# bjzhb666/GS-LoRA

Measured on AMD Instinct MI355X. Metric: forgetting-step images/sec, ViT-P8S8 d6 112px r=8, higher is better.
Workload: dtype fp16

## Files before the change

### gs-lora_amd/csrc/attention.hip

```cpp
#include <stdlib.h>

#include <algorithm>
#include <type_traits>

#include "gsl_common.h"

using namespace gsl;
#include "gsl_h16.h"
GSL_OPNS_BEGIN

typedef op16x8_t bf16x8_t;
typedef __attribute__((ext_vector_type(4))) float f32x4_t;

constexpr int HD = 64;
constexpr int KLD = 80;
__device__ __forceinline__ int lds_off(int row, int col) { return row * KLD + col; }

union Frag {
  uint4 u;
  uint2 h[2];
  bf16x8_t v;
};

__device__ __forceinline__ f32x4_t mfma16(const bf16x8_t a, const bf16x8_t b, const f32x4_t c) {
// ... 1973 lines not shown
  GSL_CHECK_ARG(qkv && o && d_o_cls && lse && dqkv && B > 0 && T > 1 && H > 0, "null/size");
  GSL_CHECK_ARG(qkv_layout >= 0 && qkv_layout <= 2 && (qkv_layout != 2 || (q_cls && dq_cls)), "qkv_layout: 0 token-major, 1 head-major, 2 kv + q_cls / dq_cls");
  const dim3 grid(B * H), blk(256);
  if (dtype == GSL_OP16)
    hipLaunchKernelGGL(attn_bwd_cls_kernel<bf16_t>, grid, blk, 0, as_stream(s), (const bf16_t*)qkv, (const bf16_t*)q_cls, (const bf16_t*)o,
                       (const bf16_t*)d_o_cls, lse, (bf16_t*)dqkv, (bf16_t*)dq_cls, T, H, scale, qkv_layout, cls_compact);
#if GSL_HAS_F32
  else if (dtype == GSL_F32)
    hipLaunchKernelGGL(attn_bwd_cls_kernel<float>, grid, blk, 0, as_stream(s), (const float*)qkv, (const float*)q_cls, (const float*)o,
                       (const float*)d_o_cls, lse, (float*)dqkv, (float*)dq_cls, T, H, scale, qkv_layout, cls_compact);
#endif
  else return fail(GSL_ERR_ARG, "gsl_attention_bwd_cls: bad dtype%s %ld", "", dtype);
  return check_launch("gsl_attention_bwd_cls");
}

#ifdef GSL_DEV
static inline int attn_env(const char* name, int dflt) { const char* e = getenv(name); return e ? atoi(e) : dflt; }
static inline unsigned long long* attn_stamps() { const char* sp = getenv("GSL_ATTN_STAMPS"); return sp ? reinterpret_cast<unsigned long long*>(strtoull(sp, nullptr, 0)) : nullptr; }
#else
static inline constexpr int attn_env(const char*, int dflt) { return dflt; }
static inline constexpr unsigned long long* attn_stamps() { return nullptr; }
#endif
static inline int attn_persistent() { return attn_env("GSL_ATTN_PERSISTENT", 1); }
static inline int attn_num_cus() {
  static int n = 0;
  if (!n) {
    int dev = 0; hipDeviceProp_t pr;
    if (hipGetDevice(&dev) == hipSuccess && hipGetDeviceProperties(&pr, dev) == hipSuccess && pr.multiProcessorCount > 0) n = pr.multiProcessorCount;
    else n = 256;
  }
// ... 127 lines not shown
```

### gs-lora_amd/csrc/gsl_h16.h

```cpp
#pragma once
#include "gsl_common.h"

extern "C" {
int h16_gsl_gemm_nt(const void* A1, int lda1, const void* W1, int ldw1, int K1, const void* A2, int lda2, const void* W2, int ldw2, int K2,
                    int M, int N, int dtype, int epilogue, float alpha, const float* bias, const void* res, const void* aux, void* out,
                    void* out2, int ldo, const float* pos, const float* cls, int T, float p_drop, uint64_t seed, uint32_t site, gsl_stream_t s);
int h16_gsl_gemm_nt_lora(const void* A, int lda, const void* W, int ldw, int K, const void* P, int ldp, const void* Q, int ldq,
                         float lora_scale, void* tout, int ldt, int M, int N, int dtype, int epilogue, const float* bias, const void* res,
                         const void* aux, void* out, void* out2, int ldo, float p_drop, uint64_t seed, uint32_t site, gsl_stream_t s);
int h16_gsl_gemm_nt_lora_mulgrad(const void* A, int lda, const void* W, int ldw, int K, const void* P, int ldp, const void* Q, int ldq,
                                 float lora_scale, void* tout, int ldt, int M, int N, const void* aux, void* out, int ldo, const void* U1,
                                 int ldu1, float* G1, long g1sn, long g1sj, const void* Y2, float* G2, long g2sn, long g2sj, int r,
                                 int accumulate, float* ws, int aux_u8, float p_drop, int dtype, const float* gscale, gsl_stream_t s);
int h16_gsl_attention_fwd(const void* qkv, void* o, float* lse, int B, int T, int H, float scale, int dtype, int qkv_layout, gsl_stream_t s);
int h16_gsl_attention_bwd(const void* qkv, const void* o, const void* d_o, const float* lse, void* dqkv, float* delta_ws, int B, int T,
                          int H, float scale, int dtype, int qkv_layout, gsl_stream_t s);
int h16_gsl_attention_fwd_cls(const void* qkv, const void* q_cls, void* o_cls, float* lse_cls, int B, int T, int H, float scale, int dtype,
                              int qkv_layout, gsl_stream_t s);
int h16_gsl_attention_bwd_cls(const void* qkv, const void* q_cls, const void* o, const void* d_o_cls, const float* lse, void* dqkv,
                              void* dq_cls, int B, int T, int H, float scale, int dtype, int qkv_layout, int cls_compact, gsl_stream_t s);
}

#ifdef GSL_OP_F16
#define GSL_FORWARD_H16(dtype, call)
#define GSL_HAS_F32 0
#else
#define GSL_FORWARD_H16(dtype, call) do { if ((dtype) == GSL_F16) return call; } while (0)
#define GSL_HAS_F32 1
#endif
```

### gs-lora_amd/gslora_hip/_lib.py

```python
import ctypes as C
import os

import contextlib

_HERE = os.path.dirname(os.path.abspath(__file__))
LIB_PATH = os.environ.get("GSLORA_HIP_LIB") or os.path.join(_HERE, "libgslora_hip.so")
DEV_LIB_PATH = os.path.join(_HERE, "libgslora_hip_dev.so")

F32, BF16, F16 = 0, 1, 2
EPI_STORE, EPI_BIAS_RES_F32, EPI_BIAS_GELU, EPI_MUL, EPI_PATCH, EPI_STORE_F32, EPI_STORE_QKV_HM, EPI_BIAS_RES_BF16, EPI_PATCH_BF16 = 0, 1, 2, 3, 4, 5, 6, 7, 8
EPI_MUL_G8, EPI_BIAS_GELU_G8, EPI_BIAS_RES_F16, EPI_PATCH_F16, EPI_STORE_LN, EPI_STORE_QKV_HM_LN = 9, 10, 11, 12, 13, 14
VERIF_FLIP_SUM, VERIF_PLAIN = 0, 1
U8_NCHW, U8_NHWC = 0, 1
NORM_SPLIT = 8
SEED_ON_DEVICE = 0x80000000

_vp, _i, _l, _f, _d, _u64, _u32 = C.c_void_p, C.c_int, C.c_long, C.c_float, C.c_double, C.c_uint64, C.c_uint32

SIGNATURES = {
    "gsl_version": [],
    "gsl_last_error": [],
    "gsl_patchify": [_vp, _vp, _i, _i, _i, _i, _i, _i, _vp],
    "gsl_unfold_patches": [_vp, _vp, _i, _i, _i, _i, _i, _i, _i, _i, _i, _vp],
    "gsl_patchify_u8": [_vp, _i, _vp, _vp, _i, _i, _i, _i, _i, _i, _vp],
    "gsl_unfold_patches_u8": [_vp, _i, _vp, _vp, _i, _i, _i, _i, _i, _i, _i, _i, _i, _vp],
    "gsl_gemm_nt": [_vp, _i, _vp, _i, _i, _vp, _i, _vp, _i, _i, _i, _i, _i, _i, _f, _vp, _vp, _vp, _vp, _vp, _i,
                    _vp, _vp, _i, _f, _u64, _u32, _vp],
    "gsl_gemm_nt_lora": [_vp, _i, _vp, _i, _i, _vp, _i, _vp, _i, _f, _vp, _i, _i, _i, _i, _i, _vp, _vp, _vp, _vp, _vp, _i,
                         _f, _u64, _u32, _vp],
    "gsl_gemm_mulgrad_ws_elems": [_i, _i, _i],
    "gsl_gemm_nt_lora_mulgrad": [_vp, _i, _vp, _i, _i, _vp, _i, _vp, _i, _f, _vp, _i, _i, _i, _vp, _vp, _i,
                                 _vp, _i, _vp, _l, _l, _vp, _vp, _l, _l, _i, _i, _vp, _i, _f, _i, _vp, _vp],
    "gsl_layernorm_fwd": [_vp, _l, _vp, _vp, _f, _vp, _vp, _vp, _i, _i, _i, _i, _vp],
    "gsl_layernorm_fwd_lora": [_vp, _l, _vp, _vp, _f, _vp, _vp, _vp, _i, _i, _vp, _i, _f, _vp, _vp],
    "gsl_layernorm_bwd": [_vp, _vp, _l, _vp, _vp, _vp, _vp, _vp, _l, _vp, _i, _i, _i, _i, _i, _f, _u64, _u32, _l, _i, _vp, _vp],
    "gsl_attention_fwd": [_vp, _vp, _vp, _i, _i, _i, _f, _i, _i, _vp],
    "gsl_attention_bwd": [_vp, _vp, _vp, _vp, _vp, _vp, _i, _i, _i, _f, _i, _i, _vp],
    "gsl_attention_fwd_cls": [_vp, _vp, _vp, _vp, _i, _i, _i, _f, _i, _i, _vp],
    "gsl_attention_bwd_cls": [_vp, _vp, _vp, _vp, _vp, _vp, _vp, _i, _i, _i, _f, _i, _i, _i, _vp],
    "gsl_lora_grad_ws_elems": [_i, _i, _i],
    "gsl_lora_grad": [_vp, _l, _vp, _i, _vp, _l, _l, _i, _i, _i, _i, _i, _vp, _vp, _vp],
    "gsl_lora_grad_batch_ws_elems": [_vp, _i],
    "gsl_lora_grad_batch": [_vp, _i, _vp, _i, _vp, _vp],
    "gsl_cosface_prep": [_vp, _vp, _i, _i, _vp],
    "gsl_head_fwd": [_vp, _i, _i, _vp, _vp, _f, _vp, _vp, _vp, _vp, _vp, _vp, _i, _i, _i, _f, _f, _vp, _i, _i, _vp],
    "gsl_head_bwd": [_vp, _vp, _vp, _i, _i, _vp, _vp, _vp, _vp, _vp, _vp, _vp, _i, _i, _i, _f, _i, _i, _f, _u64, _u32, _i, _i, _i, _vp, _vp, _i, _vp],
    "gsl_head_fwd_margin": [_vp, _i, _i, _vp, _vp, _f, _vp, _vp, _vp, _vp, _vp, _vp, _i, _i, _i, _f, _f, _vp, _i, _i, _i, _d, _i, _vp, _vp],
    "gsl_head_bwd_margin": [_vp, _vp, _vp, _i, _i, _vp, _vp, _vp, _vp, _vp, _vp, _vp, _i, _i, _i, _f, _i, _i, _f, _u64, _u32, _i, _i, _i, _vp,
                            _vp, _i, _i, _d, _i, _vp, _vp, _vp],
    "gsl_ce_fwd": [_vp, _vp, _vp, _vp, _i, _i, _vp],
    "gsl_ce_bwd": [_vp, _vp, _vp, _f, _vp, _i, _i, _i, _vp],
    "gsl_proto_kl_fwd": [_vp, _vp, _vp, _vp, _vp, _i, _i, _i, _vp],
    "gsl_loss_combine": [_vp, _vp, _vp, _vp, _vp, _vp, _vp, _f, _f, _f, _f, _f, _f, _f, _f, _vp, _vp, _vp, _vp],
    "gsl_loss_combine_pack": [_vp, _vp, _i, _f, _f, _f, _f, _f, _f, _vp, _vp, _vp, _vp],
# ... 77 lines not shown
```

### gs-lora_amd/gslora_hip/ops.py

```python
import ctypes

import torch

from . import _lib as L

ATTN_MAX_T = 1025


def check_num_tokens(model, T):
    if T > ATTN_MAX_T:
        raise NotImplementedError(f"{model}: this geometry gives {T} tokens per image; the gs-lora_amd attention kernels take at most "
                                  f"{ATTN_MAX_T} (GSL_ATTN_MAX_T: a 32 x 32 patch grid plus the cls token)")


DT = {torch.float32: L.F32, torch.bfloat16: L.BF16, torch.float16: L.F16}


def _p(t):
    return None if t is None else t.data_ptr()


def _stream():
    return torch.cuda.current_stream().cuda_stream

# ... 271 lines not shown
                                           _stream()), "gsl_attention_fwd_cls")
    return o, lse


def attention_bwd_cls(qkv, o, d_o_cls, lse, B, T, H, scale, layout=0, q_cls=None):
    _need(qkv, o, d_o_cls, lse, q_cls)
    nw = 2 if layout == 2 else 3
    dqkv = torch.empty(B * T, nw * H * 64, device=qkv.device, dtype=qkv.dtype)
    dq = torch.empty(B, H * 64, device=qkv.device, dtype=qkv.dtype) if layout == 2 else None
    compact = o.shape[0] == B and lse.dim() == 2
    L.check(L.load().gsl_attention_bwd_cls(_p(qkv), _p(q_cls), _p(o), _p(d_o_cls), _p(lse), _p(dqkv), _p(dq), B, T, H, float(scale),
                                           code(qkv.dtype), int(layout), 1 if compact else 0, _stream()), "gsl_attention_bwd_cls")
    return (dqkv, dq) if layout == 2 else dqkv




def lora_grad(Y, U, G, gsn, gsj, r, accumulate=True, gscale=None):
    if not (Y.is_cuda and U.is_cuda and Y.stride(1) == 1 and U.stride(1) == 1):
        raise RuntimeError("lora_grad: operands must be CUDA tensors with unit column stride")
    M, N = Y.shape
    lib = L.load()
    need = lib.gsl_lora_grad_ws_elems(M, N, r)
    ws = _workspace((Y.device.index,), need, Y.device, floor=1 << 22)
    L.check(lib.gsl_lora_grad(_p(Y), Y.stride(0), _p(U), U.stride(0), G.data_ptr(), gsn, gsj, M, N, r, code(Y.dtype),
                              1 if accumulate else 0, _p(ws), _p(gscale), _stream()), "gsl_lora_grad")


class _LgradDesc(ctypes.Structure):
    _fields_ = [("Y", ctypes.c_void_p), ("ldy", ctypes.c_long), ("U", ctypes.c_void_p), ("ldu", ctypes.c_int), ("M", ctypes.c_int),
# ... 435 lines not shown
```

### gs-lora_amd/gslora_hip/vit_runner.py

```python
import os

import torch

from . import _lib as L
from . import ops

PADK = 64
OP16 = (torch.bfloat16, torch.float16)
SITE_EMB = 1_000_000
GRAD_STREAM_BF16 = os.environ.get("GSLORA_GRAD_STREAM", "bf16").lower() != "f32"
FWD_STREAM = os.environ.get("GSLORA_FWD_STREAM", "f16").lower()
if FWD_STREAM not in ("f16", "bf16", "f32"):
    raise ValueError(f"GSLORA_FWD_STREAM must be f16, bf16 or f32, not {FWD_STREAM!r}")
GP8 = os.environ.get("GSLORA_GP8", "1") != "0"

FUSE_LORA_GRAD = True
TAIL_CLS = True
QSPLIT = True
INK_MIN_ROWS = 8192
LN1_FOLD = os.environ.get("GSLORA_LN1_FOLD", "1") != "0"
GRAD_TARGET_EXP = int(os.environ.get("GSLORA_GRAD_TARGET_EXP", "0"))
if GRAD_TARGET_EXP and not 4 <= GRAD_TARGET_EXP <= 15:
    raise ValueError(f"GSLORA_GRAD_TARGET_EXP={GRAD_TARGET_EXP}: 0 (default) or 4 .. 15")
INK_SMALL = True
LGRAD_BATCH_MAX_ROWS = 1 << 30
LN_LORA = False
QKV_HEAD_MAJOR = True


class BlockSpec:
    __slots__ = ("ln1", "qkv_w", "qkv_b", "out", "ln2", "l1", "l2", "qkv_lora")

    def __init__(self, ln1, qkv_w, qkv_b, out, ln2, l1, l2, qkv_lora=None):
# ... 186 lines not shown

    def w(self, name, param, dtype):
        if dtype == torch.float32:
            return param.detach()
        return self._cached(self._wcache, (name, "n", dtype), param, lambda p: ops.cast(p.contiguous(), dtype))

    def w_ln(self, name, weight, gamma, beta, bias, dtype):
        def build(weight, gamma, beta, bias=None):
            w32 = weight.float()
            wf = ops.cast((w32 * gamma.float()[None, :]).contiguous(), dtype)
            c = wf.float().sum(1).contiguous()
            d = (w32 @ beta.float()) + (bias.float() if bias is not None else 0.0)
            return wf, c, d.contiguous()
        return self._cached(self._wcache, (name, "ln", dtype), (weight, gamma, beta) + (() if bias is None else (bias,)), build)

    def w_conv(self, name, param, dtype):
        def build(p):
            w2 = p.permute(0, 2, 3, 1).reshape(p.shape[0], -1).contiguous()
            return w2 if dtype == torch.float32 else ops.cast(w2, dtype)
        return self._cached(self._wcache, (name, "conv", dtype), param, build)

    def w_kpad(self, name, param, kpad, dtype):
        def build(p):
            w2 = torch.zeros(p.shape[0], kpad, device=p.device, dtype=torch.float32)
            w2[:, :p.shape[1]] = p
            return w2 if dtype == torch.float32 else ops.cast(w2, dtype)
        return self._cached(self._wcache, (name, "kpad", kpad, dtype), param, build)

    def wT(self, name, param, dtype):
        return self._cached(self._wcache, (name, "t", dtype), param, lambda p: ops.transpose_cast(p.contiguous(), dtype))
# ... 92 lines not shown
            self._lcache.clear()
            self._retired.extend(t[0] for t in self._pack_tables.values())
            self._retired.extend(e["out"] for e in self._packs.values())
            self._packs.clear()
            self._pack_tables.clear()
        return self.bucket

    def forward(self, img, label, save):
        c, parts, u8tab, label = self._fwd_prepare(img, label, save)
        sp = c.sp
        x = self._fwd_patch(c, parts, u8tab)
        stash = []
        for i, blk in enumerate(sp.blocks):
            tail = TAIL_CLS and i == len(sp.blocks) - 1 and sp.pool == "cls"
            xn, mean1, rstd1 = self._fwd_ln1(c, blk, x)
            qkv, q_cls, uq, hm = self._fwd_qkv(c, i, blk, x, xn, mean1, rstd1, tail)
            xn_keep = xn if (c.attn_site and save) else None
            del xn
            o, lse, x1 = self._fwd_attention(c, i, blk, x, qkv, q_cls, hm, tail)
            x2, st = self._fwd_ffn(c, i, blk, x1)
            if save:
                st.update(x=x, mean1=mean1, rstd1=rstd1, qkv=qkv, qkv_hm=hm, o=o, lse=lse, x1=x1, xn=xn_keep, uq=uq, tail=tail, q_cls=q_cls)
                stash.append(st)
            x = x2
        logits, emb, head = self._fwd_head(c, x, label)
        return logits, emb, (dict(ctx=c, layers=stash, x_last=x, emb=emb, label=label, **head) if save else None)

    def _fwd_prepare(self, img, label, save):
        m = self.model
        raw = list(img) if isinstance(img, (tuple, list)) else [img]
        norm = getattr(m, "input_norm", None)
        u8 = norm is not None and all(t.dtype == torch.uint8 for t in raw)
        if norm is not None and not u8 and any(t.dtype == torch.uint8 for t in raw):
            raise ValueError(f"{type(m).__name__}: the batches of one forward must be all uint8 or all float once set_input_norm() is in effect")
        parts = raw if u8 else [t.float().contiguous() for t in raw]
        img = parts[0]
        if not all(t.is_cuda for t in parts):
# ... 69 lines not shown
        kv, q = slice(inner, None), slice(None, inner)
        epi = L.EPI_STORE_LN if fold else L.EPI_STORE
        ops.gemm_nt(a, w[kv], qkv, epilogue=epi, aux=rows(cw, kv), bias=rows(b, kv), **ln)
        q_cls = torch.empty(B, inner, device=c.dev, dtype=dt)
        ops.gemm_nt(a.view(B, T * D)[:, :D], w[q], q_cls, epilogue=epi, T=T if fold else 0,
                    aux=rows(cw, q), bias=rows(b, q), **ln)
        return qkv, q_cls, None, 2

    def _fwd_attention(self, c, i, blk, x, qkv, q_cls, hm, tail):
        sp, B, T, D = c.sp, c.B, c.T, c.D
        if tail:
            o, lse = ops.attention_fwd_cls(qkv, B, T, c.H, sp.attn_scale, layout=hm, q_cls=q_cls)
            xres = x.view(B, T, D)[:, 0].contiguous()
        else:
            o, lse = ops.attention_fwd(qkv, B, T, c.H, sp.attn_scale, layout=hm)
            xres = x
        x1 = torch.empty(xres.shape[0], D, device=c.dev, dtype=c.xdt)
        ops.gemm_nt(o, self.w(f"wo{i}", blk.out.weight, c.dt), x1, epilogue=c.epi_res,
                    bias=blk.out.bias.detach(), res=xres, p_drop=c.p_drop, seed=c.seed, site=(4 * i) | c.sflag)
        return o, lse, x1

    def _fwd_ffn(self, c, i, blk, x1):
        dt, D, r, s_lora, dev, save = c.dt, c.D, c.r, c.s_lora, c.dev, c.save
        p_drop, seed, sflag = c.p_drop, c.seed, c.sflag
        n2, l1, l2 = blk.ln2, blk.l1, blk.l2
        Mr, mlp = x1.shape[0], l1.weight.shape[0]
        lora_on = r > 0 and not c.attn_site and not l1.merged
        ln_u1 = LN_LORA and lora_on and r <= 16 and D in (512, 768) and x1.dtype == torch.bfloat16 and dt == torch.bfloat16
        if ln_u1:
            xn2, mean2, rstd2, u1_ln = ops.layernorm_fwd_lora(x1, D, Mr, D, n2.weight.detach(), n2.bias.detach(), c.eps,
                                                               self.lora_pack(f"A1_{i}", l1.lora_A, "A_rows", dt), s_lora)
        else:
            xn2, mean2, rstd2 = ops.layernorm_fwd(x1, D, Mr, D, n2.weight.detach(), n2.bias.detach(), c.eps, dt)
        if lora_on and (abs(l1.scaling * r - 1.0) > 1e-9 or abs(l2.scaling * r - 1.0) > 1e-9):
            raise NotImplementedError("gs-lora_amd: the fused LoRA path uses scaling = 1 / r (lora_alpha = 1, the only value GS-LoRA "
# ... 204 lines not shown

    def _bwd_ln2(self, c, i, blk, st, dxn2, dx, gather):
        gamma, kw = blk.ln2.weight.detach(), dict(p_drop=c.p_drop, seed=c.seed, site=(4 * i) | c.sflag, gmax=c.gmax)
        if gather:
            return ops.layernorm_bwd(dxn2, st["x1"], c.T * c.D, gamma, _cls_rows(c, st["mean2"].view(-1, 1), 1).view(-1),
                                     _cls_rows(c, st["rstd2"].view(-1, 1), 1).view(-1), dx, drop_row_stride=c.T * c.D, **kw)
        return ops.layernorm_bwd(dxn2, st["x1"], c.D, gamma, st["mean2"], st["rstd2"], dx, **kw)

    def _bwd_attention(self, c, st, d_o, sparse):
        if sparse:
            return ops.attention_bwd_cls(st["qkv"], st["o"], d_o, st["lse"], c.B, c.T, c.H, c.sp.attn_scale, layout=st["qkv_hm"], q_cls=st["q_cls"])
        return ops.attention_bwd(st["qkv"], st["o"], d_o, st["lse"], c.B, c.T, c.H, c.sp.attn_scale, layout=st["qkv_hm"])

    def _bwd_qkv_frozen(self, c, i, blk, st, d_o, sparse):
        dt, D, inner = c.dt, c.D, c.H * 64
        dxn1 = torch.empty(c.M, D, device=c.dev, dtype=dt)
        dqkv = self._bwd_attention(c, st, d_o, sparse)
        wt = self.wT(f"qkv{i}", blk.qkv_w, dt)
        if st["q_cls"] is None:
            ops.gemm_nt(dqkv, wt, dxn1)
        else:
            dkv, dq_cls = dqkv
            ops.gemm_nt(dkv, wt[:, inner:], dxn1)
            rows = dxn1.view(c.B, c.T * D)[:, :D]
            ops.gemm_nt(dq_cls, wt[:, :inner], rows, epilogue=_res_epilogue(dt), bias=self._zeros(D, c.dev), res=rows)
        return dxn1

    def _bwd_qkv_lora(self, c, i, blk, st, dqkv):
        dt, D, r, ml = c.dt, c.D, c.r, blk.qkv_lora
        qo = self.qkv_lora_ops(i, ml, dt)
        v = torch.empty(c.M, PADK, device=c.dev, dtype=dt)
        ops.gemm_nt(dqkv, qo["BblkT"], v, alpha=c.s_lora)
        ng, inner = len(ml.enable_lora), c.H * 64
# ... 11 lines not shown
```

### include/gslora_hip.h

```cpp
#ifndef GSLORA_HIP_H
#define GSLORA_HIP_H

#include <stdint.h>

#ifdef __cplusplus
extern "C" {
#endif

#define GSL_API __attribute__((visibility("default")))

typedef void* gsl_stream_t;

enum gsl_dtype { GSL_F32 = 0, GSL_BF16 = 1, GSL_F16 = 2 };

enum gsl_status {
  GSL_OK = 0,
  GSL_ERR_ARG = -1,
  GSL_ERR_LAUNCH = -2,
  GSL_ERR_UNSUPPORTED = -3
};

enum gsl_epilogue {
  GSL_EPI_STORE = 0,
  GSL_EPI_BIAS_RES_F32 = 1,
// ... 54 lines not shown
GSL_API int gsl_layernorm_fwd_lora(const void* x, long x_row_stride, const float* gamma, const float* beta, float eps, void* y,
                           float* mean, float* rstd, int M, int D, const void* P, int ldp, float alpha, void* u, gsl_stream_t s);
GSL_API int gsl_layernorm_bwd(const void* dy, const void* x, long x_row_stride, const float* gamma,
                      const float* mean, const float* rstd, const void* dres,
                      void* dx, long io_row_stride, void* dxb, int M, int D, int dtype, int stream_dtype, int x_dtype,
                      float p_drop, uint64_t seed, uint32_t site, long drop_row_stride, int dres_cls_T, float* gmax, gsl_stream_t s);

#define GSL_ATTN_MAX_T 1025
GSL_API int gsl_attention_fwd(const void* qkv, void* o, float* lse, int B, int T, int H, float scale, int dtype, int qkv_layout, gsl_stream_t s);
GSL_API int gsl_attention_bwd(const void* qkv, const void* o, const void* d_o, const float* lse, void* dqkv,
                      float* delta_ws, int B, int T, int H, float scale, int dtype, int qkv_layout, gsl_stream_t s);
GSL_API int gsl_attention_fwd_cls(const void* qkv, const void* q_cls, void* o_cls, float* lse_cls, int B, int T, int H, float scale,
                                  int dtype, int qkv_layout, gsl_stream_t s);
GSL_API int gsl_attention_bwd_cls(const void* qkv, const void* q_cls, const void* o, const void* d_o_cls, const float* lse, void* dqkv,
                                  void* dq_cls, int B, int T, int H, float scale, int dtype, int qkv_layout, int cls_compact, gsl_stream_t s);

GSL_API long gsl_lora_grad_ws_elems(int M, int N, int r);
GSL_API int gsl_lora_grad(const void* Y, long ldy, const void* U, int ldu, float* G, long gsn, long gsj,
                  int M, int N, int r, int dtype, int accumulate, float* ws, const float* gscale, gsl_stream_t s);
typedef struct gsl_lgrad_desc {
  const void* Y; long ldy; const void* U; int ldu; int M; int N; int r; int accumulate; int pad_; float* G; long gsn, gsj;
} gsl_lgrad_desc;
GSL_API long gsl_lora_grad_batch_ws_elems(const gsl_lgrad_desc* descs, int n);
GSL_API int gsl_lora_grad_batch(const gsl_lgrad_desc* descs, int n, float* ws, int dtype, const float* gscale, gsl_stream_t s);


GSL_API int gsl_cosface_prep(const float* W, float* Wn, int C, int D, gsl_stream_t s);
GSL_API int gsl_head_fwd(const void* x, int x_dtype, int T, const float* gamma, const float* beta, float eps,
                 const float* Wn, const int64_t* label, float* emb, float* mean, float* rstd,
                 float* logits, int B, int D, int C, float cos_s, float cos_m,
// ... 96 lines not shown
```

Before: 45710.

## Stream last-block CLS attention by folding K/V projections into query and output

For the tail block, where only the CLS token's output is needed, the K and V projections over all tokens are no longer materialized. The CLS query is instead projected through the K weights into model space, scored directly against the layer-normed input, softmaxed, and the probability-weighted row sum is projected through V. The backward pass mirrors this with a dedicated kernel that forms dxn via split hi/lo fp16 MFMA products. This removes the full QKV GEMM and the attention over all tokens in the last block, at the cost of new block-diagonal weight caches, extra small GEMMs, and fp16 hi/lo splitting to limit precision loss.

```diff
diff --git a/gs-lora_amd/csrc/attention.hip b/gs-lora_amd/csrc/attention.hip
--- a/gs-lora_amd/csrc/attention.hip
+++ b/gs-lora_amd/csrc/attention.hip
@@ -2011,6 +2011,297 @@
   return check_launch("gsl_attention_bwd_cls");
 }
 
+constexpr int CS_NT = 256, CS_NW = CS_NT / 64;
+constexpr int CS_TM = 224;
+constexpr int CS_DMAX = 768;
+
+__device__ __forceinline__ void cs_norm8(const uint4 u, float mu, float rs, const float4 g0, const float4 g1, const float4 b0, const float4 b1,
+                                         float v[8]) {
+  unpack2o(u.x, v[0], v[1]); unpack2o(u.y, v[2], v[3]); unpack2o(u.z, v[4], v[5]); unpack2o(u.w, v[6], v[7]);
+  v[0] = fmaf((v[0] - mu) * rs, g0.x, b0.x); v[1] = fmaf((v[1] - mu) * rs, g0.y, b0.y);
+  v[2] = fmaf((v[2] - mu) * rs, g0.z, b0.z); v[3] = fmaf((v[3] - mu) * rs, g0.w, b0.w);
+  v[4] = fmaf((v[4] - mu) * rs, g1.x, b1.x); v[5] = fmaf((v[5] - mu) * rs, g1.y, b1.y);
+  v[6] = fmaf((v[6] - mu) * rs, g1.z, b1.z); v[7] = fmaf((v[7] - mu) * rs, g1.w, b1.w);
+}
+
+constexpr float CS_LO = 256.0f;
+__device__ __forceinline__ void cs_split2(float a, float b, uint32_t& hi, uint32_t& lo) {
+  hi = pack2o(a, b);
+  float ha, hb;
+  unpack2o(hi, ha, hb);
+  lo = pack2o((a - ha) * CS_LO, (b - hb) * CS_LO);
+}
+__device__ __forceinline__ void cs_split8(const float v[8], uint4& hi, uint4& lo) {
+  cs_split2(v[0], v[1], hi.x, lo.x); cs_split2(v[2], v[3], hi.y, lo.y);
+  cs_split2(v[4], v[5], hi.z, lo.z); cs_split2(v[6], v[7], hi.w, lo.w);
+}
+
+__device__ __forceinline__ void cs_rows_dot(const op16_t* __restrict__ xb, const float* __restrict__ mean, const float* __restrict__ rstd,
+                                            const float* __restrict__ gamma, const float* __restrict__ beta, const op16_t* __restrict__ vec,
+                                            int Tn, int D, int H, float* zs) {
+  const int lane = threadIdx.x & 63, wave = threadIdx.x >> 6, fr = lane & 15, fc = lane >> 4;
+  const int ntile = (Tn + 15) >> 4;
+  for (int tile = wave; tile < ntile; tile += CS_NW) {
+    const int t = min(tile * 16 + fr, Tn - 1);
+    const float mu = mean[t], rs = rstd[t];
+    const op16_t* xr = xb + (size_t)t * D + fc * 8;
+    const op16_t* vr = vec + (size_t)min(fr, H - 1) * D + fc * 8;
+    f32x4_t acc = {0.f, 0.f, 0.f, 0.f}, acl = {0.f, 0.f, 0.f, 0.f};
+#pragma unroll 4
+    for (int k = 0; k < D; k += 32) {
+      const uint4 xv = *reinterpret_cast<const uint4*>(xr + k);
+      const float4* gp = reinterpret_cast<const float4*>(gamma + k + fc * 8);
+      const float4* bp = reinterpret_cast<const float4*>(beta + k + fc * 8);
+      float v[8];
+      cs_norm8(xv, mu, rs, gp[0], gp[1], bp[0], bp[1], v);
+      Frag a, al, b;
+      cs_split8(v, a.u, al.u);
+      b.u = *reinterpret_cast<const uint4*>(vr + k);
+      if (fr >= H) b.u = make_uint4(0, 0, 0, 0);
+      acc = mfma16(a.v, b.v, acc);
+      acl = mfma16(al.v, b.v, acl);
+    }
+    acc += acl * (1.0f / CS_LO);
+#pragma unroll
+    for (int i = 0; i < 4; ++i) zs[fr * CS_TM + tile * 16 + 4 * fc + i] = acc[i];
+  }
+}
+
+template <int HP>
+__device__ __forceinline__ void cs_weighted_rowsum(const op16_t* __restrict__ xb, const float* __restrict__ mean, const float* __restrict__ rstd,
+                                                   const float* __restrict__ gamma, const float* __restrict__ beta, const float* w, float* red,
+                                                   op16_t* __restrict__ out, int Tn, int D, int H) {
+  const int lane = threadIdx.x & 63, wave = threadIdx.x >> 6;
+  const int C = D >> 3;
+  for (int c0 = 0; c0 < C; c0 += 64) {
+    const int c = c0 + lane;
+    const bool live = c < C;
+    const int cc = live ? c : 0;
+    const float4 g0 = *reinterpret_cast<const float4*>(gamma + cc * 8), g1 = *reinterpret_cast<const float4*>(gamma + cc * 8 + 4);
+    const float4 b0 = *reinterpret_cast<const float4*>(beta + cc * 8), b1 = *reinterpret_cast<const float4*>(beta + cc * 8 + 4);
+    float acc[HP][8];
+#pragma unroll
+    for (int h = 0; h < HP; ++h)
+#pragma unroll
+      for (int i = 0; i < 8; ++i) acc[h][i] = 0.f;
+#pragma unroll 2
+    for (int t = wave; t < Tn; t += CS_NW) {
+      const uint4 xv = *reinterpret_cast<const uint4*>(xb + (size_t)t * D + cc * 8);
+      float v[8];
+      cs_norm8(xv, mean[t], rstd[t], g0, g1, b0, b1, v);
+      const float4* wr = reinterpret_cast<const float4*>(w + t * 16);
+#pragma unroll
+      for (int h4 = 0; h4 < HP / 4; ++h4) {
+        const float4 wv = wr[h4];
+        const float ws[4] = {wv.x, wv.y, wv.z, wv.w};
+#pragma unroll
+        for (int j = 0; j < 4; ++j)
+#pragma unroll
+          for (int i = 0; i < 8; ++i) acc[h4 * 4 + j][i] = fmaf(ws[j], v[i], acc[h4 * 4 + j][i]);
+      }
+    }
+#pragma unroll
+    for (int h = 0; h < HP; ++h) {
+      __syncthreads();
+      *reinterpret_cast<float4*>(red + wave * 512 + lane * 8) = make_float4(acc[h][0], acc[h][1], acc[h][2], acc[h][3]);
+      *reinterpret_cast<float4*>(red + wave * 512 + lane * 8 + 4) = make_float4(acc[h][4], acc[h][5], acc[h][6], acc[h][7]);
+      __syncthreads();
+      if (wave == (h & (CS_NW - 1)) && live && h < H) {
+        float s[8];
+#pragma unroll
+        for (int i = 0; i < 8; ++i) s[i] = red[lane * 8 + i];
+#pragma unroll
+        for (int wv = 1; wv < CS_NW; ++wv)
+#pragma unroll
+          for (int i = 0; i < 8; ++i) s[i] += red[wv * 512 + lane * 8 + i];
+        *reinterpret_cast<uint4*>(out + (size_t)h * D + c * 8) =
+            make_uint4(pack2o(s[0], s[1]), pack2o(s[2], s[3]), pack2o(s[4], s[5]), pack2o(s[6], s[7]));
+      }
+    }
+    __syncthreads();
+  }
+}
+
+template <int HP>
+__global__ __launch_bounds__(CS_NT) void attn_cls_stream_fwd_kernel(const op16_t* __restrict__ x, const float* __restrict__ mean,
+                                                                    const float* __restrict__ rstd, const float* __restrict__ gamma,
+                                                                    const float* __restrict__ beta, const op16_t* __restrict__ qt,
+                                                                    const float* __restrict__ sb, op16_t* __restrict__ y, float* __restrict__ p,
+                                                                    int Tn, int D, int H) {
+  GSL_OP16_KERNEL_ENTRY();
+  __shared__ __align__(16) float zs[16 * CS_TM];
+  __shared__ __align__(16) float pt[CS_TM * 16];
+  __shared__ __align__(16) float red[CS_NW * 512];
+  const int b = blockIdx.x, lane = threadIdx.x & 63, wave = threadIdx.x >> 6;
+  const op16_t* xb = x + (size_t)b * Tn * D;
+  const float* mb = mean + (size_t)b * Tn;
+  const float* rb = rstd + (size_t)b * Tn;
+  for (int i = threadIdx.x; i < CS_TM * 16; i += CS_NT) pt[i] = 0.f;
+  cs_rows_dot(xb, mb, rb, gamma, beta, qt + (size_t)b * H * D, Tn, D, H, zs);
+  __syncthreads();
+  for (int h = wave; h < H; h += CS_NW) {
+    const float add = sb ? sb[(size_t)b * H + h] : 0.f;
+    float s[4], m = -3.0e38f;
+#pragma unroll
+    for (int j = 0; j < 4; ++j) {
+      const int t = lane + 64 * j;
+      s[j] = t < Tn ? zs[h * CS_TM + t] + add : -3.0e38f;
+      m = fmaxf(m, s[j]);
+    }
+    m = wave_max(m);
+    float e = 0.f;
+#pragma unroll
+    for (int j = 0; j < 4; ++j) { s[j] = (lane + 64 * j < Tn) ? expf(s[j] - m) : 0.f; e += s[j]; }
+    e = wave_sum(e);
+    const float inv = 1.0f / e;
+#pragma unroll
+    for (int j = 0; j < 4; ++j) {
+      const int t = lane + 64 * j;
+      if (t < Tn) {
+        const float pv = s[j] * inv;
+        p[((size_t)b * H + h) * Tn + t] = pv;
+        pt[t * 16 + h] = pv;
+      }
+    }
+  }
+  __syncthreads();
+  cs_weighted_rowsum<HP>(xb, mb, rb, gamma, beta, pt, red, y + (size_t)b * H * D, Tn, D, H);
+}
+
+constexpr int CS_DC = 256;
+constexpr int CS_BWD_AB = CS_TM * 32 * 2, CS_BWD_R1 = (16 * CS_TM + CS_TM * 16 + CS_NW * 512) * 4;
+static_assert(CS_DC * 32 * 2 <= CS_BWD_R1, "the [qt ; dy]^T pass fits the retired region");
+constexpr int CS_BWD_LDS = 2 * CS_BWD_AB + CS_BWD_R1;
+
+template <int HP>
+__global__ __launch_bounds__(CS_NT) void attn_cls_stream_bwd_kernel(const op16_t* __restrict__ x, const float* __restrict__ mean,
+                                                                    const float* __restrict__ rstd, const float* __restrict__ gamma,
+                                                                    const float* __restrict__ beta, const op16_t* __restrict__ qt,
+                                                                    const float* __restrict__ p, const op16_t* __restrict__ dy,
+                                                                    op16_t* __restrict__ dqt, op16_t* __restrict__ dxn, int Tn, int D, int H) {
+  GSL_OP16_KERNEL_ENTRY();
+  extern __shared__ __align__(16) unsigned char cs_smem[];
+  op16_t* ab = reinterpret_cast<op16_t*>(cs_smem);
+  op16_t* abl = reinterpret_cast<op16_t*>(cs_smem + CS_BWD_AB);
+  float* zs = reinterpret_cast<float*>(cs_smem + 2 * CS_BWD_AB);
+  float* dst = zs + 16 * CS_TM;
+  float* red = dst + CS_TM * 16;
+  op16_t* bt = reinterpret_cast<op16_t*>(cs_smem + 2 * CS_BWD_AB);
+  const int b = blockIdx.x, lane = threadIdx.x & 63, wave = threadIdx.x >> 6, fr = lane & 15, fc = lane >> 4;
+  const op16_t* xb = x + (size_t)b * Tn * D;
+  const float* mb = mean + (size_t)b * Tn;
+  const float* rb = rstd + (size_t)b * Tn;
+  for (int i = threadIdx.x; i < CS_TM * 16; i += CS_NT) {
+    dst[i] = 0.f;
+    reinterpret_cast<uint32_t*>(ab)[i] = 0u;
+    reinterpret_cast<uint32_t*>(abl)[i] = 0u;
+  }
+  cs_rows_dot(xb, mb, rb, gamma, beta, dy + (size_t)b * H * D, Tn, D, H, zs);
+  __syncthreads();
+  for (int h = wave; h < H; h += CS_NW) {
+    float pv[4], dp[4], c = 0.f;
+#pragma unroll
+    for (int j = 0; j < 4; ++j) {
+      const int t = lane + 64 * j;
+      pv[j] = t < Tn ? p[((size_t)b * H + h) * Tn + t] : 0.f;
+      dp[j] = t < Tn ? zs[h * CS_TM + t] : 0.f;
+      c = fmaf(pv[j], dp[j], c);
+    }
+    c = wave_sum(c);
+#pragma unroll
+    for (int j = 0; j < 4; ++j) {
+      const int t = lane + 64 * j;
+      if (t < Tn) {
+        const float ds = pv[j] * (dp[j] - c);
+        dst[t * 16 + h] = ds;
+        uint32_t hi, lo;
+        cs_split2(ds, pv[j], hi, lo);
+        ab[t * 32 + h] = (op16_t)(hi & 0xffffu); ab[t * 32 + 16 + h] = (op16_t)(hi >> 16);
+        abl[t * 32 + h] = (op16_t)(lo & 0xffffu); abl[t * 32 + 16 + h] = (op16_t)(lo >> 16);
+      }
+    }
+  }
+  __syncthreads();
+  cs_weighted_rowsum<HP>(xb, mb, rb, gamma, beta, dst, red, dqt + (size_t)b * H * D, Tn, D, H);
+  const int ntile = (Tn + 15) >> 4;
+  for (int d0 = 0; d0 < D; d0 += CS_DC) {
+    const int dc = min(CS_DC, D - d0), Cc = dc >> 3;
+    __syncthreads();
+    for (int idx = threadIdx.x; idx < 32 * Cc; idx += CS_NT) {
+      const int k = idx / Cc, c = idx - k * Cc, hh = k & 15;
+      uint4 u = make_uint4(0, 0, 0, 0);
+      if (hh < H) u = *reinterpret_cast<const uint4*>((k < 16 ? qt : dy) + ((size_t)b * H + hh) * D + d0 + c * 8);
+      const uint32_t w4[4] = {u.x, u.y, u.z, u.w};
+#pragma unroll
+      for (int i = 0; i < 4; ++i) {
+        bt[(c * 8 + 2 * i) * 32 + k] = (op16_t)(w4[i] & 0xffffu);
+        bt[(c * 8 + 2 * i + 1) * 32 + k] = (op16_t)(w4[i] >> 16);
+      }
+    }
+    __syncthreads();
+    for (int tile = wave; tile < ntile; tile += CS_NW) {
+      const int t = tile * 16 + fr;
+      const bf16x8_t bhi = *reinterpret_cast<const bf16x8_t*>(ab + (tile * 16 + fr) * 32 + fc * 8);
+      const bf16x8_t blo = *reinterpret_cast<const bf16x8_t*>(abl + (tile * 16 + fr) * 32 + fc * 8);
+      op16_t* orow = dxn + ((size_t)b * Tn + min(t, Tn - 1)) * D + d0 + 4 * fc;
+#pragma unroll 4
+      for (int dtile = 0; dtile < (dc >> 4); ++dtile) {
+        const bf16x8_t afrag = *reinterpret_cast<const bf16x8_t*>(bt + (dtile * 16 + fr) * 32 + fc * 8);
+        const f32x4_t z = {0.f, 0.f, 0.f, 0.f};
+        f32x4_t acc = mfma16(afrag, bhi, z);
+        acc += mfma16(afrag, blo, z) * (1.0f / CS_LO);
+        if (t < Tn) store4bf(orow + dtile * 16, acc, 1.0f);
+      }
+    }
+  }
+}
+
+__global__ __launch_bounds__(256) void attn_cls_stream_sb_kernel(const op16_t* __restrict__ q_cls, const float* __restrict__ bk,
+                                                                 float* __restrict__ sb, int n, int H, float scale) {
+  GSL_OP16_KERNEL_ENTRY();
+  const int i = blockIdx.x * 256 + threadIdx.x;
+  if (i >= n) return;
+  const op16_t* q = q_cls + (size_t)i * HD;
+  const float* bb = bk + (size_t)(i % H) * HD;
+  float s = 0.f;
+  for (int j = 0; j < HD; ++j) s = fmaf(o2f(q[j]), bb[j], s);
+  sb[i] = s * scale;
+}
+
+#define GSL_CLS_STREAM_ARGS "16-bit dtype, 2 <= T <= 224, 1 <= H <= 16, D % 64 == 0, D <= 768"
+extern "C" int GSL_ENTRY(gsl_attention_cls_stream_sb)(const void* q_cls, const float* bk, float* sb, int B, int H, float scale, int dtype,
+                                                      gsl_stream_t s) {
+  GSL_FORWARD_H16(dtype, h16_gsl_attention_cls_stream_sb(q_cls, bk, sb, B, H, scale, dtype, s));
+  GSL_CHECK_ARG(q_cls && bk && sb && B > 0 && H > 0 && dtype == GSL_OP16, "null/size/16-bit dtype");
+  hipLaunchKernelGGL(attn_cls_stream_sb_kernel, dim3((B * H + 255) / 256), dim3(256), 0, as_stream(s), (const op16_t*)q_cls, bk, sb, B * H, H, scale);
+  return check_launch("gsl_attention_cls_stream_sb");
+}
+
+extern "C" int GSL_ENTRY(gsl_attention_cls_stream_fwd)(const void* x, const float* mean, const float* rstd, const float* gamma,
+                                                       const float* beta, const void* qt, const float* sb, void* y, float* p, int B, int T,
+                                                       int D, int H, int dtype, gsl_stream_t s) {
+  GSL_FORWARD_H16(dtype, h16_gsl_attention_cls_stream_fwd(x, mean, rstd, gamma, beta, qt, sb, y, p, B, T, D, H, dtype, s));
+  GSL_CHECK_ARG(x && mean && rstd && gamma && beta && qt && y && p && B > 0, "null/size");
+  GSL_CHECK_ARG(dtype == GSL_OP16 && T >= 2 && T <= CS_TM && H >= 1 && H <= 16 && (D % 64) == 0 && D > 0 && D <= CS_DMAX, GSL_CLS_STREAM_ARGS);
+  const op16_t* xx = (const op16_t*)x; const op16_t* qq = (const op16_t*)qt;
+  if (H <= 8) hipLaunchKernelGGL(attn_cls_stream_fwd_kernel<8>, dim3(B), dim3(CS_NT), 0, as_stream(s), xx, mean, rstd, gamma, beta, qq, sb, (op16_t*)y, p, T, D, H);
+  else hipLaunchKernelGGL(attn_cls_stream_fwd_kernel<16>, dim3(B), dim3(CS_NT), 0, as_stream(s), xx, mean, rstd, gamma, beta, qq, sb, (op16_t*)y, p, T, D, H);
+  return check_launch("gsl_attention_cls_stream_fwd");
+}
+
+extern "C" int GSL_ENTRY(gsl_attention_cls_stream_bwd)(const void* x, const float* mean, const float* rstd, const float* gamma,
+                                                       const float* beta, const void* qt, const float* p, const void* dy, void* dqt,
+                                                       void* dxn, int B, int T, int D, int H, int dtype, gsl_stream_t s) {
+  GSL_FORWARD_H16(dtype, h16_gsl_attention_cls_stream_bwd(x, mean, rstd, gamma, beta, qt, p, dy, dqt, dxn, B, T, D, H, dtype, s));
+  GSL_CHECK_ARG(x && mean && rstd && gamma && beta && qt && p && dy && dqt && dxn && B > 0, "null/size");
+  GSL_CHECK_ARG(dtype == GSL_OP16 && T >= 2 && T <= CS_TM && H >= 1 && H <= 16 && (D % 64) == 0 && D > 0 && D <= CS_DMAX, GSL_CLS_STREAM_ARGS);
+  const op16_t* xx = (const op16_t*)x; const op16_t* qq = (const op16_t*)qt; const op16_t* gg = (const op16_t*)dy;
+  const int lds = CS_BWD_LDS;
+  if (H <= 8) hipLaunchKernelGGL(attn_cls_stream_bwd_kernel<8>, dim3(B), dim3(CS_NT), lds, as_stream(s), xx, mean, rstd, gamma, beta, qq, p, gg, (op16_t*)dqt, (op16_t*)dxn, T, D, H);
+  else hipLaunchKernelGGL(attn_cls_stream_bwd_kernel<16>, dim3(B), dim3(CS_NT), lds, as_stream(s), xx, mean, rstd, gamma, beta, qq, p, gg, (op16_t*)dqt, (op16_t*)dxn, T, D, H);
+  return check_launch("gsl_attention_cls_stream_bwd");
+}
+
 #ifdef GSL_DEV
 static inline int attn_env(const char* name, int dflt) { const char* e = getenv(name); return e ? atoi(e) : dflt; }
 static inline unsigned long long* attn_stamps() { const char* sp = getenv("GSL_ATTN_STAMPS"); return sp ? reinterpret_cast<unsigned long long*>(strtoull(sp, nullptr, 0)) : nullptr; }
diff --git a/gs-lora_amd/csrc/gsl_h16.h b/gs-lora_amd/csrc/gsl_h16.h
--- a/gs-lora_amd/csrc/gsl_h16.h
+++ b/gs-lora_amd/csrc/gsl_h16.h
@@ -19,6 +19,12 @@
                               int qkv_layout, gsl_stream_t s);
 int h16_gsl_attention_bwd_cls(const void* qkv, const void* q_cls, const void* o, const void* d_o_cls, const float* lse, void* dqkv,
                               void* dq_cls, int B, int T, int H, float scale, int dtype, int qkv_layout, int cls_compact, gsl_stream_t s);
+int h16_gsl_attention_cls_stream_sb(const void* q_cls, const float* bk, float* sb, int B, int H, float scale, int dtype, gsl_stream_t s);
+int h16_gsl_attention_cls_stream_fwd(const void* x, const float* mean, const float* rstd, const float* gamma, const float* beta,
+                                     const void* qt, const float* sb, void* y, float* p, int B, int T, int D, int H, int dtype, gsl_stream_t s);
+int h16_gsl_attention_cls_stream_bwd(const void* x, const float* mean, const float* rstd, const float* gamma, const float* beta,
+                                     const void* qt, const float* p, const void* dy, void* dqt, void* dxn, int B, int T, int D, int H,
+                                     int dtype, gsl_stream_t s);
 }
 
 #ifdef GSL_OP_F16
diff --git a/gs-lora_amd/gslora_hip/_lib.py b/gs-lora_amd/gslora_hip/_lib.py
--- a/gs-lora_amd/gslora_hip/_lib.py
+++ b/gs-lora_amd/gslora_hip/_lib.py
@@ -38,6 +38,9 @@
     "gsl_attention_bwd": [_vp, _vp, _vp, _vp, _vp, _vp, _i, _i, _i, _f, _i, _i, _vp],
     "gsl_attention_fwd_cls": [_vp, _vp, _vp, _vp, _i, _i, _i, _f, _i, _i, _vp],
     "gsl_attention_bwd_cls": [_vp, _vp, _vp, _vp, _vp, _vp, _vp, _i, _i, _i, _f, _i, _i, _i, _vp],
+    "gsl_attention_cls_stream_sb": [_vp, _vp, _vp, _i, _i, _f, _i, _vp],
+    "gsl_attention_cls_stream_fwd": [_vp, _vp, _vp, _vp, _vp, _vp, _vp, _vp, _vp, _i, _i, _i, _i, _i, _vp],
+    "gsl_attention_cls_stream_bwd": [_vp, _vp, _vp, _vp, _vp, _vp, _vp, _vp, _vp, _vp, _i, _i, _i, _i, _i, _vp],
     "gsl_lora_grad_ws_elems": [_i, _i, _i],
     "gsl_lora_grad": [_vp, _l, _vp, _i, _vp, _l, _l, _i, _i, _i, _i, _i, _vp, _vp, _vp],
     "gsl_lora_grad_batch_ws_elems": [_vp, _i],
diff --git a/gs-lora_amd/gslora_hip/ops.py b/gs-lora_amd/gslora_hip/ops.py
--- a/gs-lora_amd/gslora_hip/ops.py
+++ b/gs-lora_amd/gslora_hip/ops.py
@@ -309,6 +309,42 @@
     return (dqkv, dq) if layout == 2 else dqkv
 
 
+CLS_STREAM_MAX_T, CLS_STREAM_MAX_D, CLS_STREAM_MAX_H = 224, 768, 16
+
+
+def attention_cls_stream_sb(q_cls, bk, H, scale):
+    _need(q_cls, bk)
+    B = q_cls.shape[0]
+    sb = torch.empty(B, H, device=q_cls.device, dtype=torch.float32)
+    L.check(L.load().gsl_attention_cls_stream_sb(_p(q_cls), _p(bk), _p(sb), B, H, float(scale), code(q_cls.dtype), _stream()),
+            "gsl_attention_cls_stream_sb")
+    return sb
+
+
+@_profiled("attn_cls_stream_fwd", lambda x, mean, rstd, gamma, beta, qt, *a, **k: (x.shape[0], x.shape[1], x.shape[0] // qt.shape[0], qt.shape[1]))
+def attention_cls_stream_fwd(x, mean, rstd, gamma, beta, qt, sb=None):
+    _need(x, mean, rstd, gamma, beta, qt, sb)
+    B, H, D = qt.shape
+    T = x.shape[0] // B
+    y = torch.empty(B, H, D, device=x.device, dtype=x.dtype)
+    p = torch.empty(B, H, T, device=x.device, dtype=torch.float32)
+    L.check(L.load().gsl_attention_cls_stream_fwd(_p(x), _p(mean), _p(rstd), _p(gamma), _p(beta), _p(qt), _p(sb), _p(y), _p(p), B, T, D, H,
+                                                  code(x.dtype), _stream()), "gsl_attention_cls_stream_fwd")
+    return y, p
+
+
+@_profiled("attn_cls_stream_bwd", lambda x, mean, rstd, gamma, beta, qt, *a, **k: (x.shape[0], x.shape[1], x.shape[0] // qt.shape[0], qt.shape[1]))
+def attention_cls_stream_bwd(x, mean, rstd, gamma, beta, qt, p, dy):
+    _need(x, mean, rstd, gamma, beta, qt, p, dy)
+    B, H, D = qt.shape
+    T = x.shape[0] // B
+    dqt = torch.empty(B, H, D, device=x.device, dtype=x.dtype)
+    dxn = torch.empty(B * T, D, device=x.device, dtype=x.dtype)
+    L.check(L.load().gsl_attention_cls_stream_bwd(_p(x), _p(mean), _p(rstd), _p(gamma), _p(beta), _p(qt), _p(p), _p(dy), _p(dqt), _p(dxn),
+                                                  B, T, D, H, code(x.dtype), _stream()), "gsl_attention_cls_stream_bwd")
+    return dqt, dxn
+
+
 
 
 def lora_grad(Y, U, G, gsn, gsj, r, accumulate=True, gscale=None):
diff --git a/gs-lora_amd/gslora_hip/vit_runner.py b/gs-lora_amd/gslora_hip/vit_runner.py
--- a/gs-lora_amd/gslora_hip/vit_runner.py
+++ b/gs-lora_amd/gslora_hip/vit_runner.py
@@ -17,6 +17,7 @@
 FUSE_LORA_GRAD = True
 TAIL_CLS = True
 QSPLIT = True
+CLS_STREAM = os.environ.get("GSLORA_CLS_STREAM", "1") != "0"
 INK_MIN_ROWS = 8192
 LN1_FOLD = os.environ.get("GSLORA_LN1_FOLD", "1") != "0"
 GRAD_TARGET_EXP = int(os.environ.get("GSLORA_GRAD_TARGET_EXP", "0"))
@@ -233,6 +234,20 @@
             return wf, c, d.contiguous()
         return self._cached(self._wcache, (name, "ln", dtype), (weight, gamma, beta) + (() if bias is None else (bias,)), build)
 
+    def w_cls_stream(self, name, weight, H, dtype):
+        def build(w):
+            inner, D = H * 64, w.shape[1]
+            w32 = w.float()
+            kbd = torch.zeros(H * D, inner, device=w.device, dtype=torch.float32)
+            vbd = torch.zeros(inner, H * D, device=w.device, dtype=torch.float32)
+            for h in range(H):
+                rows, cols = slice(h * 64, (h + 1) * 64), slice(h * D, (h + 1) * D)
+                kbd[cols, rows] = w32[inner:2 * inner][rows].t()
+                vbd[rows, cols] = w32[2 * inner:][rows]
+            cast = lambda t: ops.cast(t.contiguous(), dtype)
+            return dict(k=cast(kbd), k_t=cast(kbd.t()), v=cast(vbd), v_t=cast(vbd.t()))
+        return self._cached(self._wcache, (name, "clsbd", dtype), weight, build)
+
     def w_conv(self, name, param, dtype):
         def build(p):
             w2 = p.permute(0, 2, 3, 1).reshape(p.shape[0], -1).contiguous()
@@ -355,13 +370,20 @@
         for i, blk in enumerate(sp.blocks):
             tail = TAIL_CLS and i == len(sp.blocks) - 1 and sp.pool == "cls"
             xn, mean1, rstd1 = self._fwd_ln1(c, blk, x)
-            qkv, q_cls, uq, hm = self._fwd_qkv(c, i, blk, x, xn, mean1, rstd1, tail)
+            cs = None
+            if tail and xn is None and self._cls_stream_ok(c):
+                qkv, uq, hm, lse = None, None, 2, None
+                q_cls, o, cs = self._fwd_cls_stream(c, i, blk, x, mean1, rstd1)
+                x1 = self._fwd_out_proj(c, i, blk, x, o, tail)
+            else:
+                qkv, q_cls, uq, hm = self._fwd_qkv(c, i, blk, x, xn, mean1, rstd1, tail)
+                o, lse, x1 = self._fwd_attention(c, i, blk, x, qkv, q_cls, hm, tail)
             xn_keep = xn if (c.attn_site and save) else None
             del xn
-            o, lse, x1 = self._fwd_attention(c, i, blk, x, qkv, q_cls, hm, tail)
             x2, st = self._fwd_ffn(c, i, blk, x1)
             if save:
-                st.update(x=x, mean1=mean1, rstd1=rstd1, qkv=qkv, qkv_hm=hm, o=o, lse=lse, x1=x1, xn=xn_keep, uq=uq, tail=tail, q_cls=q_cls)
+                st.update(x=x, mean1=mean1, rstd1=rstd1, qkv=qkv, qkv_hm=hm, o=o, lse=lse, x1=x1, xn=xn_keep, uq=uq, tail=tail, q_cls=q_cls,
+                          cs=cs)
                 stash.append(st)
             x = x2
         logits, emb, head = self._fwd_head(c, x, label)
@@ -461,11 +483,36 @@
             xres = x.view(B, T, D)[:, 0].contiguous()
         else:
             o, lse = ops.attention_fwd(qkv, B, T, c.H, sp.attn_scale, layout=hm)
-            xres = x
-        x1 = torch.empty(xres.shape[0], D, device=c.dev, dtype=c.xdt)
+        return o, lse, self._fwd_out_proj(c, i, blk, x, o, tail)
+
+    def _fwd_out_proj(self, c, i, blk, x, o, tail):
+        xres = x.view(c.B, c.T, c.D)[:, 0].contiguous() if tail else x
+        x1 = torch.empty(xres.shape[0], c.D, device=c.dev, dtype=c.xdt)
         ops.gemm_nt(o, self.w(f"wo{i}", blk.out.weight, c.dt), x1, epilogue=c.epi_res,
                     bias=blk.out.bias.detach(), res=xres, p_drop=c.p_drop, seed=c.seed, site=(4 * i) | c.sflag)
-        return o, lse, x1
+        return x1
+
+    @staticmethod
+    def _cls_stream_ok(c):
+        return (CLS_STREAM and QSPLIT and not c.attn_site and c.dt in OP16 and c.H <= ops.CLS_STREAM_MAX_H and c.D % 64 == 0
+                and c.D <= ops.CLS_STREAM_MAX_D and 2 <= c.T <= ops.CLS_STREAM_MAX_T)
+
+    def _fwd_cls_stream(self, c, i, blk, x, mean1, rstd1):
+        dt, B, T, D, H, inner, scale = c.dt, c.B, c.T, c.D, c.H, c.H * 64, c.sp.attn_scale
+        w, cw, b = self.w_ln(f"qkv{i}", blk.qkv_w, blk.ln1.weight, blk.ln1.bias, blk.qkv_b, dt)
+        q_cls = torch.empty(B, inner, device=c.dev, dtype=dt)
+        ops.gemm_nt(x.view(B, T * D)[:, :D], w[:inner], q_cls, epilogue=L.EPI_STORE_LN, T=T, aux=cw[:inner], bias=b[:inner], pos=mean1, cls=rstd1)
+        bd = self.w_cls_stream(f"qkv{i}", blk.qkv_w, H, dt)
+        qt = torch.empty(B, H, D, device=c.dev, dtype=dt)
+        ops.gemm_nt(q_cls, bd["k"], qt.view(B, H * D), alpha=scale)
+        sb = bv = None
+        if blk.qkv_b is not None:
+            qb = blk.qkv_b.detach()
+            sb, bv = ops.attention_cls_stream_sb(q_cls, qb[inner:2 * inner], H, scale), qb[2 * inner:]
+        y, p = ops.attention_cls_stream_fwd(x, mean1, rstd1, blk.ln1.weight.detach(), blk.ln1.bias.detach(), qt, sb)
+        o = torch.empty(B, inner, device=c.dev, dtype=dt)
+        ops.gemm_nt(y.view(B, H * D), bd["v"], o, bias=bv)
+        return q_cls, o, dict(qt=qt, p=p)
 
     def _fwd_ffn(self, c, i, blk, x1):
         dt, D, r, s_lora, dev, save = c.dt, c.D, c.r, c.s_lora, c.dev, c.save
@@ -700,9 +747,20 @@
 
     def _bwd_qkv_frozen(self, c, i, blk, st, d_o, sparse):
         dt, D, inner = c.dt, c.D, c.H * 64
+        wt = self.wT(f"qkv{i}", blk.qkv_w, dt)
+        if st.get("cs") is not None:
+            cs, bd = st["cs"], self.w_cls_stream(f"qkv{i}", blk.qkv_w, c.H, dt)
+            dy = torch.empty(c.B, c.H, D, device=c.dev, dtype=dt)
+            ops.gemm_nt(d_o, bd["v_t"], dy.view(c.B, c.H * D))
+            dqt, dxn1 = ops.attention_cls_stream_bwd(st["x"], st["mean1"], st["rstd1"], blk.ln1.weight.detach(), blk.ln1.bias.detach(),
+                                                     cs["qt"], cs["p"], dy)
+            dq_cls = torch.empty(c.B, inner, device=c.dev, dtype=dt)
+            ops.gemm_nt(dqt.view(c.B, c.H * D), bd["k_t"], dq_cls, alpha=c.sp.attn_scale)
+            rows = dxn1.view(c.B, c.T * D)[:, :D]
+            ops.gemm_nt(dq_cls, wt[:, :inner], rows, epilogue=_res_epilogue(dt), bias=self._zeros(D, c.dev), res=rows)
+            return dxn1
         dxn1 = torch.empty(c.M, D, device=c.dev, dtype=dt)
         dqkv = self._bwd_attention(c, st, d_o, sparse)
-        wt = self.wT(f"qkv{i}", blk.qkv_w, dt)
         if st["q_cls"] is None:
             ops.gemm_nt(dqkv, wt, dxn1)
         else:
diff --git a/include/gslora_hip.h b/include/gslora_hip.h
--- a/include/gslora_hip.h
+++ b/include/gslora_hip.h
@@ -92,6 +92,12 @@
                                   int dtype, int qkv_layout, gsl_stream_t s);
 GSL_API int gsl_attention_bwd_cls(const void* qkv, const void* q_cls, const void* o, const void* d_o_cls, const float* lse, void* dqkv,
                                   void* dq_cls, int B, int T, int H, float scale, int dtype, int qkv_layout, int cls_compact, gsl_stream_t s);
+GSL_API int gsl_attention_cls_stream_sb(const void* q_cls, const float* bk, float* sb, int B, int H, float scale, int dtype, gsl_stream_t s);
+GSL_API int gsl_attention_cls_stream_fwd(const void* x, const float* mean, const float* rstd, const float* gamma, const float* beta,
+                                  const void* qt, const float* sb, void* y, float* p, int B, int T, int D, int H, int dtype, gsl_stream_t s);
+GSL_API int gsl_attention_cls_stream_bwd(const void* x, const float* mean, const float* rstd, const float* gamma, const float* beta,
+                                  const void* qt, const float* p, const void* dy, void* dqt, void* dxn, int B, int T, int D, int H,
+                                  int dtype, gsl_stream_t s);
 
 GSL_API long gsl_lora_grad_ws_elems(int M, int N, int r);
 GSL_API int gsl_lora_grad(const void* Y, long ldy, const void* U, int ldu, float* G, long gsn, long gsj,
```

After: 46110 (median of 6 runs). About the same (+0.9%).
